# LeadRDRK/ZPack

Hardware: AMD Instinct MI355X
Metric: decompressed GiB/s over all entries; % HBM roofline (higher is better)
Workload: dtype u8; 1 GPU; c2_lz4_64k; entries_per_gpu=100000, entries_total=100000, archive_image_bytes_this_rank=3543588472, archive_image_bytes_all_ranks=3543588472, method=lz4, level=0, class_mix=70/20/5/5 text/records/random/runs, parallelism=one batch per rank, no data-path collective, rehearsal_one_card=False, frames_by=liblz4/libzstd of the image, reference writer call sequence

## Files before the change

### zpack_amd/csrc/xxh3_device.h

```cpp
#pragma once
#include "zpk_device.h"

namespace zpk {

#define ZPK_P32_1 0x9E3779B1U
#define ZPK_P32_2 0x85EBCA77U
#define ZPK_P32_3 0xC2B2AE3DU
#define ZPK_P32_4 0x27D4EB2FU
#define ZPK_P32_5 0x165667B1U
#define ZPK_P64_1 0x9E3779B185EBCA87ULL
#define ZPK_P64_2 0xC2B2AE3D27D4EB4FULL
#define ZPK_P64_3 0x165667B19E3779F9ULL
#define ZPK_P64_4 0x85EBCA77C2B2AE63ULL
#define ZPK_P64_5 0x27D4EB2F165667C5ULL
#define ZPK_PMX_1 0x165667919E3779F9ULL
#define ZPK_PMX_2 0x9FB21C651E98DF25ULL

__device__ __constant__ const u8 XXH3_SECRET[192] = {
    0xb8, 0xfe, 0x6c, 0x39, 0x23, 0xa4, 0x4b, 0xbe, 0x7c, 0x01, 0x81, 0x2c, 0xf7, 0x21, 0xad, 0x1c,
    0xde, 0xd4, 0x6d, 0xe9, 0x83, 0x90, 0x97, 0xdb, 0x72, 0x40, 0xa4, 0xa4, 0xb7, 0xb3, 0x67, 0x1f,
    0xcb, 0x79, 0xe6, 0x4e, 0xcc, 0xc0, 0xe5, 0x78, 0x82, 0x5a, 0xd0, 0x7d, 0xcc, 0xff, 0x72, 0x21,
    0xb8, 0x08, 0x46, 0x74, 0xf7, 0x43, 0x24, 0x8e, 0xe0, 0x35, 0x90, 0xe6, 0x81, 0x3a, 0x26, 0x4c,
    0x3c, 0x28, 0x52, 0xbb, 0x91, 0xc3, 0x00, 0xcb, 0x88, 0xd0, 0x65, 0x8b, 0x1b, 0x53, 0x2e, 0xa3,
    0x71, 0x64, 0x48, 0x97, 0xa2, 0x0d, 0xf9, 0x4e, 0x38, 0x19, 0xef, 0x46, 0xa9, 0xde, 0xac, 0xd8,
    0xa8, 0xfa, 0x76, 0x3f, 0xe3, 0x9c, 0x34, 0x3f, 0xf9, 0xdc, 0xbb, 0xc7, 0xc7, 0x0b, 0x4f, 0x1d,
    0x8a, 0x51, 0xe0, 0x4b, 0xcd, 0xb4, 0x59, 0x31, 0xc8, 0x9f, 0x7e, 0xc9, 0xd9, 0x78, 0x73, 0x64,
    0xea, 0xc5, 0xac, 0x83, 0x34, 0xd3, 0xeb, 0xc3, 0xc5, 0x81, 0xa0, 0xff, 0xfa, 0x13, 0x63, 0xeb,
    0x17, 0x0d, 0xdd, 0x51, 0xb7, 0xf0, 0xda, 0x49, 0xd3, 0x16, 0x55, 0x26, 0x29, 0xd4, 0x68, 0x9e,
    0x2b, 0x16, 0xbe, 0x58, 0x7d, 0x47, 0xa1, 0xfc, 0x8f, 0xf8, 0xb8, 0xd1, 0x7a, 0xd0, 0x31, 0xce,
    0x45, 0xcb, 0x3a, 0x8f, 0x95, 0x16, 0x04, 0x28, 0xaf, 0xd7, 0xfb, 0xca, 0xbb, 0x4b, 0x40, 0x7e,
};

__device__ __forceinline__ u64 sec64(int off) { return ld64(XXH3_SECRET + off); }
__device__ __forceinline__ u32 sec32(int off) { return ld32(XXH3_SECRET + off); }

__device__ __forceinline__ u64 mul128_fold64(u64 a, u64 b) { return (a * b) ^ __umul64hi(a, b); }
__device__ __forceinline__ u64 xxh64_avalanche(u64 h)
{
    h ^= h >> 33; h *= ZPK_P64_2; h ^= h >> 29; h *= ZPK_P64_3; h ^= h >> 32; return h;
}
__device__ __forceinline__ u64 xxh3_avalanche(u64 h) { h ^= h >> 37; h *= ZPK_PMX_1; h ^= h >> 32; return h; }
__device__ __forceinline__ u64 bswap64(u64 x) { return __builtin_bswap64(x); }

__device__ __forceinline__ u64 xxh3_mix16(const u8* in, int soff)
{
    return mul128_fold64(ld64(in) ^ sec64(soff), ld64(in + 8) ^ sec64(soff + 8));
}

__device__ inline u64 xxh3_short(const u8* in, u32 len)
{
    if (len == 0) return xxh64_avalanche(sec64(56) ^ sec64(64));
    if (len <= 3) {
        u32 c1 = ld8(in), c2 = ld8(in + (len >> 1)), c3 = ld8(in + len - 1);
        u32 combined = (c1 << 16) | (c2 << 24) | c3 | (len << 8);
        u64 flip = (u64)(sec32(0) ^ sec32(4));
        return xxh64_avalanche((u64)combined ^ flip);
    }
    if (len <= 8) {
        u32 a = ld32(in), b = ld32(in + len - 4);
        u64 flip = sec64(8) ^ sec64(16);
        u64 in64 = (u64)b + ((u64)a << 32);
        u64 h = in64 ^ flip;
        h ^= rotl64(h, 49) ^ rotl64(h, 24);
        h *= ZPK_PMX_2;
        h ^= (h >> 35) + len;
        h *= ZPK_PMX_2;
        return h ^ (h >> 28);
    }
    if (len <= 16) {
        u64 lo = ld64(in) ^ (sec64(24) ^ sec64(32));
        u64 hi = ld64(in + len - 8) ^ (sec64(40) ^ sec64(48));
        u64 acc = len + bswap64(lo) + hi + mul128_fold64(lo, hi);
        return xxh3_avalanche(acc);
    }
    if (len <= 128) {
        u64 acc = (u64)len * ZPK_P64_1;
        if (len > 32) {
            if (len > 64) {
                if (len > 96) {
                    acc += xxh3_mix16(in + 48, 96);
                    acc += xxh3_mix16(in + len - 64, 112);
                }
                acc += xxh3_mix16(in + 32, 64);
                acc += xxh3_mix16(in + len - 48, 80);
            }
            acc += xxh3_mix16(in + 16, 32);
            acc += xxh3_mix16(in + len - 32, 48);
        }
        acc += xxh3_mix16(in, 0);
        acc += xxh3_mix16(in + len - 16, 16);
        return xxh3_avalanche(acc);
    }
    u64 acc = (u64)len * ZPK_P64_1;
    u32 rounds = len / 16;
    for (u32 i = 0; i < 8; i++) acc += xxh3_mix16(in + 16 * i, 16 * (int)i);
    acc = xxh3_avalanche(acc);
    for (u32 i = 8; i < rounds; i++) acc += xxh3_mix16(in + 16 * i, 16 * (int)(i - 8) + 3);
    acc += xxh3_mix16(in + len - 16, 136 - 17);
    return xxh3_avalanche(acc);
}


struct Xxh3Wave {
    u64 a0, a1;
    u64 k0, k1;
    u64 s0, s1;

    __device__ __forceinline__ void init(int lane)
    {
        const int q = lane & 3, s = lane >> 2;
        const u64 init[8] = { ZPK_P32_3, ZPK_P64_1, ZPK_P64_2, ZPK_P64_3, ZPK_P64_4, ZPK_P32_2, ZPK_P64_5, ZPK_P32_1 };
        a0 = q == 0 ? init[0] : q == 1 ? init[2] : q == 2 ? init[4] : init[6];
        a1 = q == 0 ? init[1] : q == 1 ? init[3] : q == 2 ? init[5] : init[7];
        k0 = sec64(8 * s + 16 * q); k1 = sec64(8 * s + 16 * q + 8);
        s0 = sec64(128 + 16 * q);   s1 = sec64(128 + 16 * q + 8);
    }

    static __device__ __forceinline__ void slot(u64 d0, u64 d1, u64 key0, u64 key1, u64& c0, u64& c1)
    {
        u64 x0 = d0 ^ key0, x1 = d1 ^ key1;
        c0 = (u64)(u32)x0 * (u64)(u32)(x0 >> 32) + d1;
        c1 = (u64)(u32)x1 * (u64)(u32)(x1 >> 32) + d0;
    }

    template <int CTRL>
    static __device__ __forceinline__ u64 add_rotated(u64 c)
    {
        const u32 rl = (u32)__builtin_amdgcn_update_dpp(0, (int)(u32)c, CTRL, 0xf, 0xf, false);
        const u32 rh = (u32)__builtin_amdgcn_update_dpp(0, (int)(u32)(c >> 32), CTRL, 0xf, 0xf, false);
        return c + (((u64)rh << 32) | rl);
    }
    static __device__ __forceinline__ u64 add_rows(u64 c)
    {
        const u32 lo = (u32)c, hi = (u32)(c >> 32);
        auto l16 = __builtin_amdgcn_permlane16_swap(lo, lo, false, false);
        auto h16 = __builtin_amdgcn_permlane16_swap(hi, hi, false, false);
        const u64 s = (((u64)h16[0] << 32) | l16[0]) + (((u64)h16[1] << 32) | l16[1]);
        const u32 slo = (u32)s, shi = (u32)(s >> 32);
        auto l32 = __builtin_amdgcn_permlane32_swap(slo, slo, false, false);
        auto h32 = __builtin_amdgcn_permlane32_swap(shi, shi, false, false);
        return (((u64)h32[0] << 32) | l32[0]) + (((u64)h32[1] << 32) | l32[1]);
    }
    template <bool NO_LDS>
    static __device__ __forceinline__ void reduce16(u64& c0, u64& c1)
    {
        if (!NO_LDS) {
            #pragma unroll
            for (int m = 4; m < 64; m <<= 1) { c0 += shfl_xor64(c0, m); c1 += shfl_xor64(c1, m); }
        } else {
            c0 = add_rotated<0x124>(c0); c1 = add_rotated<0x124>(c1);
            c0 = add_rotated<0x128>(c0); c1 = add_rotated<0x128>(c1);
            c0 = add_rows(c0); c1 = add_rows(c1);
        }
    }

    __device__ __forceinline__ void scramble()
    {
        a0 = ((a0 ^ (a0 >> 47)) ^ s0) * ZPK_P32_1;
        a1 = ((a1 ^ (a1 >> 47)) ^ s1) * ZPK_P32_1;
    }

    __device__ __forceinline__ void block(u128 d)
    {
        u64 c0, c1;
        slot(d.lo, d.hi, k0, k1, c0, c1);
        reduce16<false>(c0, c1);
        a0 += c0; a1 += c1;
        scramble();
    }

    __device__ __forceinline__ u64 finish(const u8* p, u32 nstripes, const u8* end, u64 total_len, int lane)
    {
        const int q = lane & 3, s = lane >> 2;
        u64 c0 = 0, c1 = 0;
        if ((u32)s < nstripes) {
            u128 d = ld128(p + 16 * lane);
            slot(d.lo, d.hi, k0, k1, c0, c1);
        } else if (s == 15) {
            u128 d = ld128(end - 64 + 16 * q);
            slot(d.lo, d.hi, sec64(121 + 16 * q), sec64(121 + 16 * q + 8), c0, c1);
        }
        reduce16<false>(c0, c1);
        a0 += c0; a1 += c1;
        u64 t = mul128_fold64(a0 ^ sec64(11 + 16 * q), a1 ^ sec64(11 + 16 * q + 8));
        t += shfl_xor64(t, 1);
        t += shfl_xor64(t, 2);
        return xxh3_avalanche(total_len * ZPK_P64_1 + t);
    }
};

struct Xxh3Lite {
    u64 a0, a1;
    __device__ __forceinline__ void init(int lane)
    {
        Xxh3Wave w; w.init(lane); a0 = w.a0; a1 = w.a1;
    }
    __device__ __forceinline__ void block(u128 d, int lane, lds_cp8 sec = nullptr)
    {
        const int q = lane & 3, s = lane >> 2;
        u64 k0, k1, s0, s1;
        if (sec) {
            k0 = ((const ZPK_LDS u64*)(sec + 8 * s + 16 * q))[0]; k1 = ((const ZPK_LDS u64*)(sec + 8 * s + 16 * q))[1];
            s0 = ((const ZPK_LDS u64*)(sec + 128 + 16 * q))[0];   s1 = ((const ZPK_LDS u64*)(sec + 128 + 16 * q))[1];
        } else { k0 = sec64(8 * s + 16 * q); k1 = sec64(8 * s + 16 * q + 8); s0 = sec64(128 + 16 * q); s1 = sec64(128 + 16 * q + 8); }
        u64 c0, c1;
        Xxh3Wave::slot(d.lo, d.hi, k0, k1, c0, c1);
        Xxh3Wave::reduce16<true>(c0, c1);
        a0 += c0; a1 += c1;
        a0 = ((a0 ^ (a0 >> 47)) ^ s0) * ZPK_P32_1;
        a1 = ((a1 ^ (a1 >> 47)) ^ s1) * ZPK_P32_1;
    }
    __device__ __forceinline__ u64 finish(const u8* p, u32 nstripes, const u8* end, u64 total_len, int lane)
    {
        Xxh3Wave w; w.init(lane); w.a0 = a0; w.a1 = a1;
        return w.finish(p, nstripes, end, total_len, lane);
    }
};

__device__ __forceinline__ u64 xxh3_64_wave(const u8* p, u64 len, int lane)
{
    if (len <= 240) {
        u64 h = 0;
        lane0_guard();
        if (lane == 0) h = xxh3_short(p, (u32)len);
        return uni64(h);
    }
    Xxh3Wave st;
    st.init(lane);
    const u64 nblocks = (len - 1) >> 10;
    const u8* q = p + 16 * lane;
    if (nblocks > 0) {
        const u64 last = nblocks - 1;
        #define XXH3_LD(i) ld128(q + (((i) < last ? (i) : last) << 10))
        u128 a0 = XXH3_LD(0), a1 = XXH3_LD(1);
        for (u64 b = 0; b < nblocks; b += 4) {
            const u128 c0 = XXH3_LD(b + 2), c1 = XXH3_LD(b + 3);
            st.block(a0);
            if (b + 1 < nblocks) st.block(a1);
            a0 = XXH3_LD(b + 4); a1 = XXH3_LD(b + 5);
            if (b + 2 < nblocks) st.block(c0);
            if (b + 3 < nblocks) st.block(c1);
        }
        #undef XXH3_LD
    }
    const u32 nstripes = (u32)(((len - 1) - (nblocks << 10)) >> 6);
    return st.finish(p + (nblocks << 10), nstripes, p + len, len, lane);
}


__device__ inline u32 xxh32_serial(const u8* p, u64 len, u32 seed)
{
    const u8* end = p + len;
    u32 h;
    if (len >= 16) {
        u32 v1 = seed + ZPK_P32_1 + ZPK_P32_2, v2 = seed + ZPK_P32_2, v3 = seed, v4 = seed - ZPK_P32_1;
        do {
            v1 = rotl32(v1 + ld32(p) * ZPK_P32_2, 13) * ZPK_P32_1;
            v2 = rotl32(v2 + ld32(p + 4) * ZPK_P32_2, 13) * ZPK_P32_1;
            v3 = rotl32(v3 + ld32(p + 8) * ZPK_P32_2, 13) * ZPK_P32_1;
            v4 = rotl32(v4 + ld32(p + 12) * ZPK_P32_2, 13) * ZPK_P32_1;
            p += 16;
        } while (p + 16 <= end);
        h = rotl32(v1, 1) + rotl32(v2, 7) + rotl32(v3, 12) + rotl32(v4, 18);
    } else {
        h = seed + ZPK_P32_5;
    }
    h += (u32)len;
    while (p + 4 <= end) { h = rotl32(h + ld32(p) * ZPK_P32_3, 17) * ZPK_P32_4; p += 4; }
    while (p < end) { h = rotl32(h + (u32)ld8(p) * ZPK_P32_5, 11) * ZPK_P32_1; p++; }
    h ^= h >> 15; h *= ZPK_P32_2; h ^= h >> 13; h *= ZPK_P32_3; h ^= h >> 16;
    return h;
}

__device__ __forceinline__ u64 xxh64_round(u64 acc, u64 in) { return rotl64(acc + in * ZPK_P64_2, 31) * ZPK_P64_1; }

__device__ inline u64 xxh64_serial(const u8* p, u64 len, u64 seed)
{
    const u8* end = p + len;
    u64 h;
    if (len >= 32) {
        u64 v1 = seed + ZPK_P64_1 + ZPK_P64_2, v2 = seed + ZPK_P64_2, v3 = seed, v4 = seed - ZPK_P64_1;
        do {
            v1 = xxh64_round(v1, ld64(p)); v2 = xxh64_round(v2, ld64(p + 8));
            v3 = xxh64_round(v3, ld64(p + 16)); v4 = xxh64_round(v4, ld64(p + 24));
            p += 32;
        } while (p + 32 <= end);
        h = rotl64(v1, 1) + rotl64(v2, 7) + rotl64(v3, 12) + rotl64(v4, 18);
        h = (h ^ xxh64_round(0, v1)) * ZPK_P64_1 + ZPK_P64_4;
        h = (h ^ xxh64_round(0, v2)) * ZPK_P64_1 + ZPK_P64_4;
        h = (h ^ xxh64_round(0, v3)) * ZPK_P64_1 + ZPK_P64_4;
        h = (h ^ xxh64_round(0, v4)) * ZPK_P64_1 + ZPK_P64_4;
    } else {
        h = seed + ZPK_P64_5;
    }
    h += len;
    while (p + 8 <= end) { h ^= xxh64_round(0, ld64(p)); h = rotl64(h, 27) * ZPK_P64_1 + ZPK_P64_4; p += 8; }
    if (p + 4 <= end) { h ^= (u64)ld32(p) * ZPK_P64_1; h = rotl64(h, 23) * ZPK_P64_2 + ZPK_P64_3; p += 4; }
    while (p < end) { h ^= (u64)ld8(p) * ZPK_P64_5; h = rotl64(h, 11) * ZPK_P64_1; p++; }
    return xxh64_avalanche(h);
}

}
```

### zpack_amd/csrc/zpk_codec.hip

```cpp
#include <hip/hip_runtime.h>
#include <stdio.h>
#include <stdlib.h>
#include <string.h>
#include <new>
#include <time.h>
#include <pthread.h>
#include <thread>
#include <atomic>
#include <vector>
#include <algorithm>


#include "zpk_device.h"
#include "xxh3_device.h"
#include "xxh3_span.h"
#include "lz4_wave.h"
#include "lx_ring.h"
#ifndef LX_WAVES_PER_SIMD
#define LX_WAVES_PER_SIMD 6
#endif
#include "zstd_wg.h"
#include "zstd_fse4.h"
#include "zstd_ring.h"
#include "lz4_pj.h"
#include "zstd_pj.h"
#include "host_walk.h"

using namespace zpk;

enum { L_NONE = 0, L_ZSTD = 1, L_LZ4 = 2, L_COUNT = 4, N_LISTS = 3, L_LZ4_RUNS = 100 ,
       L_LZ4_GEN = 101  };
enum { C_ZSTD_TWO_STAGE = 9, C_ZSTD_FUSED = 10, C_EXEC_HEAD = 16, C_LEFT_COUNT = 17,
       C_RETRY_LZ4 = 18, C_RETRY_ZSTD = 19,
       C_RETRY_HEAD = 20,
       C_LZ4_LEFT = 21, C_LZ4_LEFT_HEAD = 22,
       C_LZ4_GEN = 3, C_LZ4_GEN_HEAD = 7,
       C_LZ4_HANDED_HEAD = 23, C_LZ4_HANDED = 24,
       C_LZ4_RETRY_HEAD = 25,
       C_ENC_CLASS = 28,
       C_ORDER_SPAN = 26,
       C_ORDER = 32,
       N_COUNTERS = 32 + 96 };
enum { S_LZ4_HANDED = N_LISTS + 5, S_LZ4_GEN = N_LISTS + 6, S_LZ4_GEN_ORDERED = N_LISTS + 7, N_LISTS_ALLOC = N_LISTS + 8 };
#define N_ORDERED 3
__device__ __forceinline__ int order_list_slot(int y) { return y == 0 ? (int)L_ZSTD : y == 1 ? (int)L_LZ4 : (int)S_LZ4_GEN; }
__device__ __forceinline__ int order_count_word(int y) { return y == 0 ? (int)L_ZSTD : y == 1 ? (int)L_LZ4 : (int)C_LZ4_GEN; }
__device__ __forceinline__ int order_out_slot(int y) { return y == 2 ? (int)S_LZ4_GEN_ORDERED : (int)N_LISTS + 3 + y; }


#define ORD_CLASSES 16
__device__ __forceinline__ int order_class(u64 size)
{
    const int lg = 63 - __clzll((long long)(size | 1));
    const int b = 26 - lg;
    return b < 0 ? 0 : (b > ORD_CLASSES - 1 ? ORD_CLASSES - 1 : b);
}
__device__ __forceinline__ int order_fast(u64 size, u64 comp) { return comp * 16 >= size * 15 ? 1 : 0; }
__device__ __forceinline__ bool lz4_header_is_plain(const u8* __restrict__ p, u64 comp_size)
{
    if (comp_size < 11) return false;
    const u32 magic = (u32)p[0] | ((u32)p[1] << 8) | ((u32)p[2] << 16) | ((u32)p[3] << 24), flg = p[4], bd = p[5];
    return magic == 0x184D2204u && (flg & 0xD7u) == 0x40u && (bd & 0x8Fu) == 0 && ((bd >> 4) & 7u) >= 4u;
}
__global__ __launch_bounds__(256) void k_classify(const u8* __restrict__ src, const zpk_decode_desc* __restrict__ desc, u64 n, u64 src_size, u64 dst_size,
                                                  zpk_decode_result* __restrict__ res, u32* __restrict__ lists, u64 list_stride,
                                                  u32* __restrict__ counters)
{
    u64 i = (u64)blockIdx.x * blockDim.x + threadIdx.x;
    const bool live = i < n;
    zpk_decode_desc d; memset(&d, 0, sizeof(d));
    if (live) d = desc[i];
    zpk_decode_result r; r.status = R_OK; r.detail = 0; r.produced = 0; r.hash = 0;
    int list = -1;
    if (!live) list = -1;
    else if (d.comp_size == 0) r.status = R_OK;
    else if (d.dst_capacity < d.uncomp_size) r.status = R_BUFFER_TOO_SMALL;
    else if (d.src_offset + d.comp_size >= src_size || d.src_offset > src_size || d.comp_size > src_size - d.src_offset)
        r.status = R_FILE_OFFSET_INVALID;
    else if (d.dst_offset > dst_size || d.dst_capacity > dst_size - d.dst_offset) { r.status = R_BUFFER_TOO_SMALL; r.detail = 0xBAD0D57u; }
    else if (d.method == ZPK_METHOD_NONE) {
        if (d.uncomp_size > d.comp_size) r.status = R_FILE_SIZE_INVALID;
        else list = L_NONE;
    }
    else if (d.method == ZPK_METHOD_ZSTD) list = L_ZSTD;
    else if (d.method == ZPK_METHOD_LZ4)
        list = d.comp_size < (d.uncomp_size >> 3) ? L_LZ4_RUNS : lz4_header_is_plain(src + d.src_offset, d.comp_size) ? L_LZ4 : L_LZ4_GEN;
    else r.status = R_COMP_METHOD_INVALID;
    if (list >= 0) { r.status = R_DECOMPRESS_FAILED; r.detail = 0xFFFFFFFFu; }
    if (live) res[i] = r;
    const int lane = lane_id();
    {
        const bool dec = list == L_ZSTD || list == L_LZ4 || list == L_LZ4_GEN;
        u32 hi = dec ? (u32)order_class(d.uncomp_size) + 1u : 0u, inv = dec ? (u32)(ORD_CLASSES - order_class(d.uncomp_size)) : 0u;
        #pragma unroll
        for (int m = 1; m < 64; m <<= 1) { const u32 a = (u32)__shfl_xor((int)hi, m, 64), b2 = (u32)__shfl_xor((int)inv, m, 64); hi = a > hi ? a : hi; inv = b2 > inv ? b2 : inv; }
        if (lane == 0 && hi) { atomicMax(&counters[C_ORDER_SPAN], hi - 1u); atomicMax(&counters[C_ORDER_SPAN + 1], inv - 1u); }
    }
    #pragma unroll
    for (int L = 0; L < N_LISTS; L++) {
        const u64 m = __ballot(list == L);
        if (m == 0) continue;
        const int leader = __ffsll((long long)m) - 1;
        u32 base = 0;
        if (lane == leader) base = atomicAdd(&counters[L], (u32)__popcll(m));
        base = (u32)__shfl((int)base, leader, 64);
        if (list == L) lists[(u64)L * list_stride + base + (u32)__popcll(m & ((1ull << lane) - 1))] = (u32)i;
    }
    {
        const u64 m = __ballot(list == L_LZ4_RUNS);
        if (m != 0) {
            const int leader = __ffsll((long long)m) - 1;
            u32 base = 0;
            if (lane == leader) base = atomicAdd(&counters[C_LZ4_LEFT], (u32)__popcll(m));
            base = (u32)__shfl((int)base, leader, 64);
            if (list == L_LZ4_RUNS) lists[(u64)(N_LISTS + 2) * list_stride + base + (u32)__popcll(m & ((1ull << lane) - 1))] = (u32)i;
        }
    }
    {
        const u64 m = __ballot(list == L_LZ4_GEN);
        if (m != 0) {
            const int leader = __ffsll((long long)m) - 1;
            u32 base = 0;
            if (lane == leader) base = atomicAdd(&counters[C_LZ4_GEN], (u32)__popcll(m));
            base = (u32)__shfl((int)base, leader, 64);
            if (list == L_LZ4_GEN) lists[(u64)S_LZ4_GEN * list_stride + base + (u32)__popcll(m & ((1ull << lane) - 1))] = (u32)i;
        }
    }
}

__device__ __forceinline__ bool order_single_class(const u32* counters) { return counters[C_ORDER_SPAN] + counters[C_ORDER_SPAN + 1] == ORD_CLASSES - 1; }
__device__ __forceinline__ void order_wave_rank(int b, int lane, u32& rank, u32& count)
{
    rank = 0; count = 0;
    u64 todo = __ballot(b >= 0);
    while (todo) {
        const int cls = __shfl(b, __ffsll((long long)todo) - 1, 64);
        const u64 m = __ballot(b == cls);
        if (b == cls) { rank = (u32)__popcll(m & ((1ull << lane) - 1)); count = (u32)__popcll(m); }
        todo &= ~m;
    }
}
__global__ __launch_bounds__(256) void k_order_count(const zpk_decode_desc* __restrict__ desc, const u32* __restrict__ lists, u64 list_stride,
                                                     u32* __restrict__ counters, int fast_last)
{
    __shared__ u32 h[ORD_CLASSES];
    const int L = order_list_slot(blockIdx.y);
    const u32 cnt = counters[order_count_word(blockIdx.y)];
    const bool uniform = order_single_class(counters);
    if ((u64)blockIdx.x * 256 >= cnt || (uniform && !fast_last)) return;
    if (threadIdx.x < ORD_CLASSES) h[threadIdx.x] = 0;
    __syncthreads();
    const u64 k = (u64)blockIdx.x * 256 + threadIdx.x;
    const int lane = lane_id();
    int b = -1;
    if (k < cnt) { const zpk_decode_desc& d = desc[lists[(u64)L * list_stride + k]]; b = uniform ? order_fast(d.uncomp_size, d.comp_size) : order_class(d.uncomp_size); }
    u32 rank, count;
    order_wave_rank(b, lane, rank, count);
    if (b >= 0 && rank == 0) atomicAdd(&h[b], count);
    __syncthreads();
    if (threadIdx.x < ORD_CLASSES && h[threadIdx.x]) atomicAdd(&counters[C_ORDER + blockIdx.y * ORD_CLASSES + threadIdx.x], h[threadIdx.x]);
}
__global__ __launch_bounds__(256) void k_order_fill(const zpk_decode_desc* __restrict__ desc, const u32* __restrict__ lists, u64 list_stride,
                                                    u32* __restrict__ all_lists , u32* __restrict__ counters, int fast_last)
{
    __shared__ u32 wcount[4][ORD_CLASSES], base[ORD_CLASSES];
    const int L = order_list_slot(blockIdx.y);
    const u32 cnt = counters[order_count_word(blockIdx.y)];
    u32* const ordered = all_lists + (u64)order_out_slot(blockIdx.y) * list_stride;
    if ((u64)blockIdx.x * 256 >= cnt) return;
    const u64 k = (u64)blockIdx.x * 256 + threadIdx.x;
    const bool uniform = order_single_class(counters);
    if (uniform && !fast_last) { if (k < cnt) ordered[k] = lists[(u64)L * list_stride + k]; return; }
    if (threadIdx.x < 4 * ORD_CLASSES) (&wcount[0][0])[threadIdx.x] = 0;
    __syncthreads();
    const int lane = lane_id(), w = threadIdx.x >> 6;
    u32 e = 0; int b = -1;
    if (k < cnt) { e = lists[(u64)L * list_stride + k]; b = uniform ? order_fast(desc[e].uncomp_size, desc[e].comp_size) : order_class(desc[e].uncomp_size); }
    u32 rank, count;
    order_wave_rank(b, lane, rank, count);
    if (b >= 0 && rank == 0) wcount[w][b] = count;
    __syncthreads();
    if (threadIdx.x < ORD_CLASSES) {
        const int c = threadIdx.x;
        const u32 total = wcount[0][c] + wcount[1][c] + wcount[2][c] + wcount[3][c];
        const u32* const hist = counters + C_ORDER + blockIdx.y * ORD_CLASSES;
        u32 before = 0;
        for (int j = 0; j < c; j++) before += hist[j];
        base[c] = total ? before + atomicAdd(&counters[C_ORDER + N_ORDERED * ORD_CLASSES + blockIdx.y * ORD_CLASSES + c], total) : 0;
    }
    __syncthreads();
    if (b >= 0) {
        u32 at = base[b] + rank;
        for (int j = 0; j < w; j++) at += wcount[j][b];
        ordered[at] = e;
    }
}

__device__ __forceinline__ bool my_slot(const u32* counters, int list, u32& idx)
{
    idx = uni((u32)(((u64)blockIdx.x * blockDim.x + threadIdx.x) >> 6));
    return idx < uni(counters[list]);
}

__device__ __forceinline__ void finish_entry(const zpk_decode_desc& d, zpk_decode_result* res, u32 e, int status, u32 detail,
                                             u64 produced, const u8* out, int lane)
{
    u64 h = 0;
    lane0_guard();
    if (status == R_OK) {
        wave_mem_fence();
#ifndef ZPK_ABL_NOHASH
        h = xxh3_64_wave(out, d.uncomp_size, lane);
#endif
        if (h != d.expect_hash && !(d.flags & ZPK_DF_SKIP_HASH)) status = R_FILE_HASH_MISMATCH;
    }
    lane0_guard();
    if (lane == 0) {
        zpk_decode_result r; r.status = status; r.detail = detail; r.produced = produced; r.hash = h;
        res[e] = r;
    }
}

__global__ __launch_bounds__(256) void k_stored(const u8* __restrict__ src, const zpk_decode_desc* __restrict__ desc,
                                                u8* __restrict__ dst, zpk_decode_result* __restrict__ res,
                                                const u32* __restrict__ list, const u32* __restrict__ counters)
{
    const int lane = lane_id();
    u32 idx;
    if (my_slot(counters, L_NONE, idx)) {
        const u32 e = uni(list[idx]);
        const zpk_decode_desc d = desc[e];
        const u8* in = uni_ptr(src + d.src_offset);
        u8* out = uni_ptr(dst + d.dst_offset);
        const u64 len = uni64(d.uncomp_size);
        u64 h;
        if (len <= 240) {
            for (u64 i = lane; i < len; i += WAVE) st8(out + i, ld8(in + i));
            h = 0;
            lane0_guard();
            if (lane == 0) h = xxh3_short(in, (u32)len);
            h = uni64(h);
        } else {
            Xxh3Wave st; st.init(lane);
            const u64 nblocks = (len - 1) >> 10;
            const u8* q = in + 16 * lane;
            u8* o = out + 16 * lane;
            u128 cur = {0, 0};
            if (nblocks) cur = ld128(q);
            for (u64 b = 0; b < nblocks; b++) {
                u128 nxt = {0, 0};
                if (b + 1 < nblocks) nxt = ld128(q + ((b + 1) << 10));
                st128(o + (b << 10), cur);
                st.block(cur);
                cur = nxt;
            }
            const u64 done = nblocks << 10;
            for (u64 i = done + lane; i < len; i += WAVE) st8(out + i, ld8(in + i));
            const u32 nstripes = (u32)(((len - 1) - done) >> 6);
            h = st.finish(in + done, nstripes, in + len, len, lane);
        }
        int status = R_OK;
        if (!(d.flags & ZPK_DF_SKIP_HASH) && h != d.expect_hash) status = R_FILE_HASH_MISMATCH;
        lane0_guard();
        if (lane == 0) {
            zpk_decode_result r; r.status = status; r.detail = 0; r.produced = len; r.hash = h;
            res[e] = r;
        }
    }
}

__device__ __forceinline__ void lz4_stats_out(u64* __restrict__ dbg, u32 e, const SeqStats& stt, u64 t_all, int lane)
{
#ifdef ZPK_STATS
    if (dbg && lane == 0) {
        u64* g = dbg + (u64)e * 8;
        g[0] = stt.t_parse; g[1] = stt.t_lit; g[2] = stt.t_dep; g[3] = stt.t_rounds;
        g[4] = ((u64)stt.batches << 32) | stt.rounds; g[5] = ((u64)stt.coops << 32) | stt.asm_batches; g[6] = SEQ_T() - t_all;
        g[7] = ((u64)stt.fix_iters << 32) | stt.chunks;
#ifdef ZPK_STATS_PARSE
        g[0] = stt.t_stage; g[1] = stt.t_walk1; g[2] = stt.t_fix; g[3] = stt.t_emit; g[4] = stt.t_tok;
        g[5] = ((u64)stt.hops_first << 32) | stt.hops_fix; g[6] = stt.slow_hops;
#endif
    }
#else
    (void)dbg; (void)e; (void)stt; (void)t_all; (void)lane;
#endif
}

template <int COOP>
__device__ __forceinline__ void lz4_entry_wave(Lz4WaveShared& shw, const u8* __restrict__ src, const u8* read_lo, const u8* read_hi,
                                               const zpk_decode_desc* __restrict__ desc, u8* dst, zpk_decode_result* __restrict__ res,
                                               u32 e, u32* __restrict__ counters, u64* __restrict__ dbg, u32* __restrict__ retry_list,
                                               u32 wd_scale, int lane)
{
    const zpk_decode_desc d = desc[e];
    const u8* in = uni_ptr(src + d.src_offset);
    u8* out = uni_ptr(dst + d.dst_offset);
    Watchdog wd; wd.arm(uni64(d.comp_size) + uni64(d.dst_capacity), wd_scale);
    SeqStats stt = {};
    const u64 t_all = SEQ_T(); (void)t_all;
    DecodeOut o = lz4f_decode_wave<COOP>(shw, wd, stt, in, uni64(d.comp_size), read_lo, read_hi, out, uni64(d.dst_capacity), lane);
    lz4_stats_out(dbg, e, stt, t_all, lane);
    if (wd.fired && retry_list) {
        lane0_guard();
        if (lane == 0) retry_list[atomicAdd(&counters[C_RETRY_LZ4], 1u)] = e;
        return;
    }
    int status = R_OK;
    if (o.rc == D_MALFORMED) status = R_DECOMPRESS_FAILED;
    else if (o.rc == D_TRUNCATED) status = o.produced < d.dst_capacity ? R_FILE_INCOMPLETE : R_BUFFER_TOO_SMALL;
    else if (o.rc == D_DST_FULL) status = R_BUFFER_TOO_SMALL;
    finish_entry(d, res, e, status, wd.fired ? 0xDEADu : (u32)(-o.rc), o.produced, out, lane);
}

__device__ __forceinline__ void lz4_entry_plain(Lz4WaveShared& shw, const u8* __restrict__ src, const u8* read_hi,
                                                const zpk_decode_desc* __restrict__ desc, u8* dst, zpk_decode_result* __restrict__ res,
                                                u32 e, u32* __restrict__ counters, u64* __restrict__ dbg, u32* __restrict__ retry_list,
                                                u32* __restrict__ handed_list, u32 wd_scale, int lane)
{
    const zpk_decode_desc& d = desc[e];
    const u8* in = uni_ptr(src + d.src_offset);
    u8* out = uni_ptr(dst + d.dst_offset);
    Watchdog wd; wd.arm(uni64(d.comp_size) + uni64(d.dst_capacity), wd_scale);
    SeqStats stt = {};
    const u64 t_all = SEQ_T(); (void)t_all;
    const bool done = lz4f_plain_wave<0>(shw, wd, stt, in, uni64(d.comp_size), read_hi, out, uni64(d.dst_capacity), uni64(d.uncomp_size), lane);
    lz4_stats_out(dbg, e, stt, t_all, lane);
    if (!done) {
        lane0_guard();
        if (lane == 0) {
            if (wd.fired) retry_list[atomicAdd(&counters[C_RETRY_LZ4], 1u)] = e;
            else handed_list[atomicAdd(&counters[C_LZ4_HANDED], 1u)] = e;
        }
        return;
    }
    finish_entry(d, res, e, R_OK, 0u, uni64(d.uncomp_size), out, lane);
}

__global__ __launch_bounds__(64, 8) void k_lz4_wave(const u8* __restrict__ src, const u8* read_hi,
                                                  const zpk_decode_desc* __restrict__ desc, u8* dst,
                                                  zpk_decode_result* __restrict__ res, const u32* __restrict__ list,
                                                  u32* __restrict__ counters, u32* __restrict__ retry_list, u32* __restrict__ handed_list
#ifdef ZPK_DEVELOPER
                                                  , u64* __restrict__ dbg, u32 wd_scale
#endif
                                                  )
{
#ifndef ZPK_DEVELOPER
    const u32 wd_scale = 1u;
    u64* const dbg = nullptr;
#endif
    const int lane = lane_id();
    __shared__ Lz4WaveShared shw;
    u32 idx;
    if (my_slot(counters, L_LZ4, idx))
        lz4_entry_plain(shw, src, read_hi, desc, dst, res, uni(list[idx]), counters, dbg, retry_list, handed_list, wd_scale, lane);
}

#ifdef ZPK_DEVELOPER
__global__ __launch_bounds__(256) void k_lz4_hand_all(const u32* __restrict__ list, u32* __restrict__ counters, u32* __restrict__ handed_list)
{
    const u64 i = (u64)blockIdx.x * blockDim.x + threadIdx.x;
    if (i < counters[L_LZ4]) handed_list[atomicAdd(&counters[C_LZ4_HANDED], 1u)] = list[i];
}
#endif

#define LZ4_GENERAL_GRID_MAX 8192u
__global__ __launch_bounds__(64, 8) void k_lz4_general(const u8* __restrict__ src, const u8* read_lo, const u8* read_hi,
                                                     const zpk_decode_desc* __restrict__ desc, u8* dst,
                                                     zpk_decode_result* __restrict__ res, const u32* __restrict__ list,
                                                     u32* __restrict__ counters, u64* __restrict__ dbg, u32* __restrict__ retry_list, u32 wd_scale)
{
    const int lane = lane_id();
    __shared__ Lz4WaveShared shw;
    const u32 n_slots = uni(counters[C_LZ4_GEN]);
    if (n_slots == 0) return;
    for (;;) {
        lane0_guard();
        u32 v = 0;
        if (lane == 0) v = atomicAdd(&counters[C_LZ4_GEN_HEAD], 1u);
        const u32 idx = uni(v);
        lane0_guard();
        if (idx >= n_slots) break;
        lz4_entry_wave<0>(shw, src, read_lo, read_hi, desc, dst, res, uni(list[idx]), counters, dbg, retry_list, wd_scale, lane);
    }
}

__global__ __launch_bounds__(64, 8) void k_lz4_retry(const u8* __restrict__ src, const u8* read_lo, const u8* read_hi,
                                                   const zpk_decode_desc* __restrict__ desc, u8* dst,
                                                   zpk_decode_result* __restrict__ res, const u32* __restrict__ lists, u64 list_stride,
                                                   u32* __restrict__ counters, u64* __restrict__ dbg, int gen_slot)
{
    const int lane = lane_id();
    __shared__ Lz4WaveShared shw;
    for (int k = 0; k < 3; k++) {
        const int count_word = k == 0 ? (int)C_LZ4_GEN : k == 1 ? (int)C_LZ4_HANDED : (int)C_RETRY_LZ4;
        const int head_word = k == 0 ? (int)C_LZ4_GEN_HEAD : k == 1 ? (int)C_LZ4_HANDED_HEAD : (int)C_LZ4_RETRY_HEAD;
        const u32* const list = lists + (u64)(k == 0 ? gen_slot : k == 1 ? (int)S_LZ4_HANDED : (int)N_LISTS) * list_stride;
        const u32 n_slots = uni(counters[count_word]);
        if (n_slots == 0 || uni(counters[head_word]) >= n_slots) continue;
        for (;;) {
            lane0_guard();
            u32 v = 0;
            if (lane == 0) v = atomicAdd(&counters[head_word], 1u);
            const u32 idx = uni(v);
            lane0_guard();
            if (idx >= n_slots) break;
            lz4_entry_wave<2>(shw, src, read_lo, read_hi, desc, dst, res, uni(list[idx]), counters, dbg, nullptr, (u32)ZPK_WATCHDOG_RETRY_SCALE, lane);
        }
    }
}

#define LZ4_LEFT_GRID_MAX 8192u
#ifndef LZ4_LEFT_WAVES
#define LZ4_LEFT_WAVES 8
#endif
__global__ __launch_bounds__(64, LZ4_LEFT_WAVES) void k_lz4_left(const u8* __restrict__ src, const u8* read_lo, const u8* read_hi,
                                                  const zpk_decode_desc* __restrict__ desc, u8* dst,
                                                  zpk_decode_result* __restrict__ res, const u32* __restrict__ list,
                                                  u32* __restrict__ counters, u64* __restrict__ dbg, u32* __restrict__ retry_list, u32 wd_scale)
{
    const int lane = lane_id();
    __shared__ Lz4WaveShared shw;
    const u32 n_slots = uni(counters[C_LZ4_LEFT]);
    if (n_slots == 0) return;
    for (;;) {
        lane0_guard();
        u32 v = 0;
        if (lane == 0) v = atomicAdd(&counters[C_LZ4_LEFT_HEAD], 1u);
        const u32 idx = uni(v);
        lane0_guard();
        if (idx >= n_slots) break;
        lz4_entry_wave<2>(shw, src, read_lo, read_hi, desc, dst, res, uni(list[idx]), counters, dbg, retry_list, wd_scale, lane);
    }
}

#define ZSTD_EXEC_GRID_MAX 4096
#ifndef ZSTD_EXEC_WAVES
#define ZSTD_EXEC_WAVES 4
#endif
#ifndef ZSTD_EXEC_DIRECT
#define ZSTD_EXEC_RING 1
#endif
__global__ __launch_bounds__(ZSTD_WG_THREADS, ZSTD_EXEC_WAVES) void k_zstd_exec(const u8* __restrict__ src, const zpk_decode_desc* __restrict__ desc,
                                                               u8* dst, zpk_decode_result* __restrict__ res,
                                                               const u32* __restrict__ list, u32* __restrict__ counters,
                                                               u8* __restrict__ lit_scratch, const u64* __restrict__ arena,
                                                               u32* __restrict__ zstate, u32* __restrict__ leftover, u64* __restrict__ dbg)
{
    const int lane = lane_id();
    const u32 nz = uni(counters[L_ZSTD]);
    if (nz == 0) return;
#ifndef ZSTD_EXEC_RING
    __shared__ __attribute__((aligned(16))) u8 sh_raw[ZSTD_SHARED_EXEC_BYTES];
    ZstdShared& sh = *(ZstdShared*)sh_raw;
    if (threadIdx.x == 0) { sh.defaults_built = 0; sh.huf_valid = 0; }
#else
    __shared__ ZstdRingShared sh;
    if (threadIdx.x == 0) sh.huf_valid = 0;
#endif
    __syncthreads();
    u8* lit = lit_scratch + (u64)blockIdx.x * ZSTD_LIT_SCRATCH;
    for (;;) {
        lane0_guard();
        u32 v = 0;
        if (lane == 0) v = atomicAdd(&counters[C_EXEC_HEAD], 1u);
        const u32 idx = uni(v);
        lane0_guard();
        if (idx >= nz) break;
        const u32 e = uni(list[idx]);
        if (uni(zstate[e]) != 1u) {
            lane0_guard();
            if (lane == 0) leftover[atomicAdd(&counters[C_LEFT_COUNT], 1u)] = e;
            lane0_guard();
            continue;
        }
        const zpk_decode_desc d = desc[e];
        const u8* in = uni_ptr(src + d.src_offset);
        u8* out = uni_ptr(dst + d.dst_offset);
        const u64* const pre = arena + (((u64)d.dst_offset + 7) >> 3);
        Watchdog wd; wd.arm(uni64(d.comp_size) + uni64(d.dst_capacity));
#ifndef ZSTD_EXEC_RING
#ifdef ZPK_STATS
        ZstdStats zs = {};
        const u64 t_all = SEQ_T();
        DecodeOut o = zstd_decode_wave<true>(sh, wd, in, uni64(d.comp_size), out, uni64(d.dst_capacity), lit, lane, &zs, pre);
        const u64 t_dec = SEQ_T();
#else
        (void)dbg;
        DecodeOut o = zstd_decode_wave<true>(sh, wd, in, uni64(d.comp_size), out, uni64(d.dst_capacity), lit, lane, nullptr, pre);
#endif
        bool ok = o.rc == D_OK;
        u64 h = 0;
        lane0_guard();
        if (ok) {
            wave_mem_fence();
    #ifndef ZPK_ABL_NOHASH
        h = xxh3_64_wave(out, d.uncomp_size, lane);
#endif
            ok = h == d.expect_hash || (d.flags & ZPK_DF_SKIP_HASH);
        }
        const int ok_status = R_OK;
#ifdef ZPK_STATS
        if (dbg && lane == 0) {
            u64* g = dbg + (u64)e * 16;
            g[0] = zs.t_lit; g[1] = zs.t_tab; g[2] = zs.t_fse; g[3] = zs.t_exec; g[4] = zs.nseq; g[5] = zs.nblk; g[6] = t_dec - t_all; g[7] = SEQ_T() - t_dec;
        }
#endif
#else
        (void)dbg;
        struct { int rc; u64 produced; } o;
        const LxResult xr = zstd_ring_decode_wave(sh, wd, in, uni64(d.comp_size), out, uni64(d.dst_capacity), uni64(d.uncomp_size), lit, pre, lane,
                                                   dbg ? dbg + (u64)e * 16 : nullptr);
        o.rc = xr.rc == LX_OK ? D_OK : -(0x100 + xr.rc); o.produced = xr.produced;
        const u64 h = xr.hash;
        const bool ok = xr.rc == LX_OK && xr.produced == uni64(d.uncomp_size);
        const int ok_status = (h == d.expect_hash || (d.flags & ZPK_DF_SKIP_HASH)) ? R_OK : R_FILE_HASH_MISMATCH;
#endif
        lane0_guard();
        if (lane == 0) {
            if (ok) {
                zpk_decode_result r; r.status = ok_status; r.detail = 0; r.produced = o.produced; r.hash = h;
                res[e] = r;
                zstate[e] = 2u;
                atomicAdd(&counters[C_ZSTD_TWO_STAGE], 1u);
            } else {
                leftover[atomicAdd(&counters[C_LEFT_COUNT], 1u)] = e;
                atomicAdd(&counters[14], 1u); counters[15] = ((u32)(-o.rc) & 0xFFFFu);
            }
        }
    }
}

__global__ __launch_bounds__(ZSTD_WG_THREADS, 3) void k_zstd(const u8* __restrict__ src, const zpk_decode_desc* __restrict__ desc,
                                                          u8* dst, zpk_decode_result* __restrict__ res,
                                                          const u32* __restrict__ list, u32* __restrict__ counters,
                                                          u8* __restrict__ lit_scratch, u64* __restrict__ dbg, int count_word,
                                                          int head_word, u32* __restrict__ retry_list, int retry_word, u32 wd_scale)
{
    const int lane = lane_id();
    const u32 nz = uni(counters[count_word]);
    if (nz == 0) return;
    __shared__ ZstdShared sh;
    if (threadIdx.x == 0) { sh.defaults_built = 0; sh.huf_valid = 0; }
    __syncthreads();
    u8* lit = lit_scratch + (u64)blockIdx.x * ZSTD_LIT_SCRATCH;
    for (;;) {
        lane0_guard();
        u32 v = 0;
        if (lane == 0) v = atomicAdd(&counters[head_word], 1u);
        const u32 idx = uni(v);
        lane0_guard();
        if (idx >= nz) break;
        const u32 e = uni(list[idx]);
        const zpk_decode_desc d = desc[e];
        const u8* in = uni_ptr(src + d.src_offset);
        u8* out = uni_ptr(dst + d.dst_offset);
        Watchdog wd; wd.arm(uni64(d.comp_size) + uni64(d.dst_capacity), wd_scale);
#ifdef ZPK_STATS
        ZstdStats zs = {};
        const u64 t_all = SEQ_T();
        DecodeOut o = zstd_decode_wave<false>(sh, wd, in, uni64(d.comp_size), out, uni64(d.dst_capacity), lit, lane, &zs);
        if (dbg && lane == 0) {
            u64* g = dbg + (u64)e * 8;
            g[0] = zs.t_lit; g[1] = zs.t_tab; g[2] = zs.t_fse; g[3] = zs.t_exec; g[4] = zs.nseq; g[5] = zs.nblk; g[6] = SEQ_T() - t_all; g[7] = 0;
        }
#else
        (void)dbg;
        DecodeOut o = zstd_decode_wave<false>(sh, wd, in, uni64(d.comp_size), out, uni64(d.dst_capacity), lit, lane);
#endif
        int status = o.rc == D_OK ? R_OK : R_DECOMPRESS_FAILED;
        if (wd.fired && retry_list) {
            lane0_guard();
            if (lane == 0) retry_list[atomicAdd(&counters[retry_word], 1u)] = e;
            lane0_guard();
            continue;
        }
        finish_entry(d, res, e, status, wd.fired ? 0xDEADu : (u32)(-o.rc), o.produced, out, lane);
        lane0_guard();
        if (lane == 0) atomicAdd(&counters[C_ZSTD_FUSED], 1u);
    }
}

__global__ __launch_bounds__(256) void k_hash(const u8* __restrict__ src, const u64* __restrict__ offsets,
                                              const u64* __restrict__ sizes, u64 n, u64* __restrict__ hashes)
{
    const int lane = lane_id();
    const u64 w = uni64(((u64)blockIdx.x * blockDim.x + threadIdx.x) >> 6);
    if (w < n) {
        u64 h = xxh3_64_wave(uni_ptr(src + offsets[w]), uni64(sizes[w]), lane);
        lane0_guard();
        if (lane == 0) hashes[w] = h;
    }
}


#define ZPK_DEC_SPLIT_MIN_DEFAULT (256ull << 10)
#define ZPK_ENC_SPLIT_MIN_DEFAULT (2ull << 20)
#define ZPK_ENC_PIECE (512u << 10)
#ifndef ZPK_PJ_CHUNK_BLOCKS
#define ZPK_PJ_CHUNK_BLOCKS 512u
#endif
#define ZPK_PJ_MAX_CHUNKS 64u
struct zpk_codec {
    int device = 0;
    hipStream_t stream = nullptr;
    pthread_mutex_t mu;
    u32* d_counters = nullptr;
    u32* d_lists = nullptr;      u64 list_cap = 0;
    u8*  d_lit = nullptr;        u64 lit_cap = 0;
    u8*  d_src = nullptr;        u64 src_cap = 0;
    u8*  h_pin[2] = {nullptr, nullptr};
    hipEvent_t pin_ev[2] = {nullptr, nullptr};
    hipStream_t s_up = nullptr, s_dn = nullptr;
    hipStream_t s_side = nullptr;
    hipEvent_t ev_fork = nullptr, ev_join = nullptr;
    void* d_pj_blocks = nullptr; u64 pj_blocks_cap = 0;
    void* d_pj_recs = nullptr;   u64 pj_recs_cap = 0;
    void* d_pj_masks = nullptr;  u64 pj_masks_cap = 0;
    void* d_pj_S = nullptr;      u64 pj_S_cap = 0;
    u32*  d_pj_flags = nullptr;
    u8*   h_bigsrc = nullptr; u64 h_bigsrc_cap = 0;
    u8*   d_big1 = nullptr;
    u32   zpj_last_err = 0;
    void* d_zpj_blocks = nullptr; u64 zpj_blocks_cap = 0;
    void* d_zpj_aux = nullptr;    u64 zpj_aux_cap = 0;
    void* d_zpj_pos = nullptr;    u64 zpj_pos_cap = 0;
    hipStream_t s_left = nullptr;
    hipEvent_t ev_lfork = nullptr, ev_ljoin = nullptr;
    volatile u32* h_seen = nullptr;
    hipEvent_t pipe_ev[2 * 64] = {};
    u8*  d_dst = nullptr;        u64 dst_cap = 0;
    void* d_desc = nullptr;      u64 desc_cap = 0;
    void* d_res = nullptr;       u64 res_cap = 0;
    u64* d_dbg = nullptr;        u64 dbg_cap = 0;
    u64* d_seq = nullptr;        u64 seq_cap = 0;
    u8*  d_pack = nullptr;       u64 pack_cap = 0;
    u8*  d_packed = nullptr;     u64 packed_cap = 0;
    u8*  d_packoff = nullptr;    u64 packoff_cap = 0;
// ... 1301 lines not shown
```

Measured before the change: 646.2 GiB/s.

## Restructure wave XXH3 to hash four blocks per iteration with row-wise reduction

The wave-level XXH3 hash now maps each 16-lane row to a different 1 KiB block, so one group iteration covers four blocks. Each lane accumulates products locally, reduces within its row using lean DPP adds, and broadcasts the four row sums with ds_bpermute before folding them into the accumulator in order. This replaces the per-block full-wave xor-shuffle reduction. In the LZ4 paths the secret keys are staged once into the LDS stage buffer instead of being reloaded. The aim is to cut reduction and synchronisation cost on the hash that runs after each decoded entry. The cost is extra LDS traffic, more complex tail handling for partial groups, and reuse of the shared stage buffer, which must not be live at that point.

```diff
diff --git a/zpack_amd/csrc/xxh3_device.h b/zpack_amd/csrc/xxh3_device.h
--- a/zpack_amd/csrc/xxh3_device.h
+++ b/zpack_amd/csrc/xxh3_device.h
@@ -106,15 +106,20 @@
     u64 k0, k1;
     u64 s0, s1;
 
-    __device__ __forceinline__ void init(int lane)
-    {
-        const int q = lane & 3, s = lane >> 2;
+    __device__ __forceinline__ void init_acc(int lane)
+    {
+        const int q = lane & 3;
         const u64 init[8] = { ZPK_P32_3, ZPK_P64_1, ZPK_P64_2, ZPK_P64_3, ZPK_P64_4, ZPK_P32_2, ZPK_P64_5, ZPK_P32_1 };
         a0 = q == 0 ? init[0] : q == 1 ? init[2] : q == 2 ? init[4] : init[6];
         a1 = q == 0 ? init[1] : q == 1 ? init[3] : q == 2 ? init[5] : init[7];
+        s0 = sec64(128 + 16 * q);   s1 = sec64(128 + 16 * q + 8);
+    }
+    __device__ __forceinline__ void init_keys(int lane)
+    {
+        const int q = lane & 3, s = lane >> 2;
         k0 = sec64(8 * s + 16 * q); k1 = sec64(8 * s + 16 * q + 8);
-        s0 = sec64(128 + 16 * q);   s1 = sec64(128 + 16 * q + 8);
-    }
+    }
+    __device__ __forceinline__ void init(int lane) { init_acc(lane); init_keys(lane); }
 
     static __device__ __forceinline__ void slot(u64 d0, u64 d1, u64 key0, u64 key1, u64& c0, u64& c1)
     {
@@ -123,12 +128,18 @@
         c1 = (u64)(u32)x1 * (u64)(u32)(x1 >> 32) + d0;
     }
 
-    template <int CTRL>
+    static __device__ __forceinline__ u64 pair64(u32 lo, u32 hi)
+    {
+        u64 v = ((u64)hi << 32) | lo;
+        asm volatile("" : "+v"(v));
+        return v;
+    }
+    template <int CTRL, bool LEAN = false>
     static __device__ __forceinline__ u64 add_rotated(u64 c)
     {
-        const u32 rl = (u32)__builtin_amdgcn_update_dpp(0, (int)(u32)c, CTRL, 0xf, 0xf, false);
-        const u32 rh = (u32)__builtin_amdgcn_update_dpp(0, (int)(u32)(c >> 32), CTRL, 0xf, 0xf, false);
-        return c + (((u64)rh << 32) | rl);
+        const u32 rl = (u32)__builtin_amdgcn_update_dpp(0, (int)(u32)c, CTRL, 0xf, 0xf, LEAN);
+        const u32 rh = (u32)__builtin_amdgcn_update_dpp(0, (int)(u32)(c >> 32), CTRL, 0xf, 0xf, LEAN);
+        return c + (LEAN ? pair64(rl, rh) : (((u64)rh << 32) | rl));
     }
     static __device__ __forceinline__ u64 add_rows(u64 c)
     {
@@ -167,6 +178,50 @@
         reduce16<false>(c0, c1);
         a0 += c0; a1 += c1;
         scramble();
+    }
+
+    static __device__ __forceinline__ void quad_keys(int lane, int it, u64& key0, u64& key1)
+    {
+        const int off = 32 * it + 8 * ((lane >> 2) & 3) + 16 * (lane & 3);
+        key0 = sec64(off); key1 = sec64(off + 8);
+    }
+    static __device__ __forceinline__ void quad_keys(lds_cp8 sec, int lane, int it, u64& key0, u64& key1)
+    {
+        const ZPK_LDS u64* w = (const ZPK_LDS u64*)(sec + 8 * ((lane >> 2) & 3) + 16 * (lane & 3)) + 4 * it;
+        key0 = w[0]; key1 = w[1];
+    }
+    static __device__ __forceinline__ void stage_secret(lds_p8 sec, int lane)
+    {
+        wave_mem_fence();
+        if (lane < 12) lds_st128(sec + 16 * lane, ld128(XXH3_SECRET + 16 * lane));
+        wave_mem_fence();
+    }
+    static __device__ __forceinline__ void quad_slot(u128 d, u64 key0, u64 key1, u64& t0, u64& t1)
+    {
+        u64 c0, c1;
+        slot(d.lo, d.hi, key0, key1, c0, c1);
+        t0 += c0; t1 += c1;
+    }
+    static __device__ __forceinline__ void row_sum(u64& t0, u64& t1)
+    {
+        t0 = add_rotated<0x124, true>(t0); t1 = add_rotated<0x124, true>(t1);
+        t0 = add_rotated<0x128, true>(t0); t1 = add_rotated<0x128, true>(t1);
+    }
+    template <int R>
+    static __device__ __forceinline__ u64 row_bcast_lds(u64 v, int l15x4)
+    {
+        const u32 lo = (u32)__builtin_amdgcn_ds_bpermute(l15x4 + 64 * R, (int)(u32)v);
+        const u32 hi = (u32)__builtin_amdgcn_ds_bpermute(l15x4 + 64 * R, (int)(u32)(v >> 32));
+        return pair64(lo, hi);
+    }
+    __device__ __forceinline__ void fold(u64 S0, u64 S1) { a0 += S0; a1 += S1; scramble(); }
+    __device__ __forceinline__ void fold_rows(u64 t0, u64 t1, u32 n, int lane)
+    {
+        const int l15x4 = 4 * (lane & 15);
+        fold(row_bcast_lds<0>(t0, l15x4), row_bcast_lds<0>(t1, l15x4));
+        if (n > 1) fold(row_bcast_lds<1>(t0, l15x4), row_bcast_lds<1>(t1, l15x4));
+        if (n > 2) fold(row_bcast_lds<2>(t0, l15x4), row_bcast_lds<2>(t1, l15x4));
+        if (n > 3) fold(row_bcast_lds<3>(t0, l15x4), row_bcast_lds<3>(t1, l15x4));
     }
 
     __device__ __forceinline__ u64 finish(const u8* p, u32 nstripes, const u8* end, u64 total_len, int lane)
@@ -217,7 +272,8 @@
     }
 };
 
-__device__ __forceinline__ u64 xxh3_64_wave(const u8* p, u64 len, int lane)
+template <bool LDS_KEYS = false>
+__device__ __forceinline__ u64 xxh3_64_wave(const u8* p, u64 len, int lane, lds_p8 sec = nullptr)
 {
     if (len <= 240) {
         u64 h = 0;
@@ -226,23 +282,42 @@
         return uni64(h);
     }
     Xxh3Wave st;
-    st.init(lane);
-    const u64 nblocks = (len - 1) >> 10;
-    const u8* q = p + 16 * lane;
+    st.init_acc(lane);
+    const u64 nblocks = uni64((len - 1) >> 10);
     if (nblocks > 0) {
-        const u64 last = nblocks - 1;
-        #define XXH3_LD(i) ld128(q + (((i) < last ? (i) : last) << 10))
-        u128 a0 = XXH3_LD(0), a1 = XXH3_LD(1);
-        for (u64 b = 0; b < nblocks; b += 4) {
-            const u128 c0 = XXH3_LD(b + 2), c1 = XXH3_LD(b + 3);
-            st.block(a0);
-            if (b + 1 < nblocks) st.block(a1);
-            a0 = XXH3_LD(b + 4); a1 = XXH3_LD(b + 5);
-            if (b + 2 < nblocks) st.block(c0);
-            if (b + 3 < nblocks) st.block(c1);
+        const u64 lastg = (nblocks - 1) >> 2;
+        const u32 nlast = (((u32)nblocks - 1u) & 3u) + 1u;
+        const u32 row = (u32)lane >> 4, l16 = 16u * ((u32)lane & 15u);
+        u64 kc[4][2] = {};
+        if (LDS_KEYS) Xxh3Wave::stage_secret(sec, lane);
+        else { Xxh3Wave::quad_keys(lane, 0, kc[0][0], kc[0][1]); Xxh3Wave::quad_keys(lane, 1, kc[1][0], kc[1][1]);
+               Xxh3Wave::quad_keys(lane, 2, kc[2][0], kc[2][1]); Xxh3Wave::quad_keys(lane, 3, kc[3][0], kc[3][1]); }
+        #define XXH3_SLOT(d, it) do { u64 k0_ = kc[it][0], k1_ = kc[it][1]; if (LDS_KEYS) Xxh3Wave::quad_keys((lds_cp8)sec, lane, it, k0_, k1_); \
+                                      Xxh3Wave::quad_slot(d, k0_, k1_, t0, t1); } while (0)
+        const u32 off_full = (row << 10) + l16, off_last = ((row < nlast ? row : nlast - 1u) << 10) + l16;
+        #define XXH3_LD(g, it) ld128(p + ((g) << 12) + ((g) == lastg ? off_last : off_full) + 256u * (it))
+        u128 a0 = XXH3_LD((u64)0, 0), a1 = XXH3_LD((u64)0, 1);
+        #pragma clang loop unroll(disable)
+        for (u64 g = 0; g <= lastg; g++) {
+            const u128 c0 = XXH3_LD(g, 2), c1 = XXH3_LD(g, 3);
+            __builtin_amdgcn_sched_barrier(0);
+            u64 t0 = 0, t1 = 0;
+            XXH3_SLOT(a0, 0);
+            XXH3_SLOT(a1, 1);
+            const u64 gn = g < lastg ? g + 1 : lastg;
+            asm volatile("" : "+v"(t0), "+v"(t1));
+            __builtin_amdgcn_sched_barrier(0);
+            a0 = XXH3_LD(gn, 0); a1 = XXH3_LD(gn, 1);
+            __builtin_amdgcn_sched_barrier(0);
+            XXH3_SLOT(c0, 2);
+            XXH3_SLOT(c1, 3);
+            Xxh3Wave::row_sum(t0, t1);
+            st.fold_rows(t0, t1, g == lastg ? nlast : 4u, lane);
         }
         #undef XXH3_LD
-    }
+        #undef XXH3_SLOT
+    }
+    st.init_keys(lane);
     const u32 nstripes = (u32)(((len - 1) - (nblocks << 10)) >> 6);
     return st.finish(p + (nblocks << 10), nstripes, p + len, len, lane);
 }
diff --git a/zpack_amd/csrc/zpk_codec.hip b/zpack_amd/csrc/zpk_codec.hip
--- a/zpack_amd/csrc/zpk_codec.hip
+++ b/zpack_amd/csrc/zpk_codec.hip
@@ -202,15 +202,16 @@
     return idx < uni(counters[list]);
 }
 
+template <bool LDS_KEYS = false>
 __device__ __forceinline__ void finish_entry(const zpk_decode_desc& d, zpk_decode_result* res, u32 e, int status, u32 detail,
-                                             u64 produced, const u8* out, int lane)
+                                             u64 produced, const u8* out, int lane, lds_p8 sec = nullptr)
 {
     u64 h = 0;
     lane0_guard();
     if (status == R_OK) {
         wave_mem_fence();
 #ifndef ZPK_ABL_NOHASH
-        h = xxh3_64_wave(out, d.uncomp_size, lane);
+        h = xxh3_64_wave<LDS_KEYS>(out, d.uncomp_size, lane, sec);
 #endif
         if (h != d.expect_hash && !(d.flags & ZPK_DF_SKIP_HASH)) status = R_FILE_HASH_MISMATCH;
     }
@@ -310,7 +311,7 @@
     if (o.rc == D_MALFORMED) status = R_DECOMPRESS_FAILED;
     else if (o.rc == D_TRUNCATED) status = o.produced < d.dst_capacity ? R_FILE_INCOMPLETE : R_BUFFER_TOO_SMALL;
     else if (o.rc == D_DST_FULL) status = R_BUFFER_TOO_SMALL;
-    finish_entry(d, res, e, status, wd.fired ? 0xDEADu : (u32)(-o.rc), o.produced, out, lane);
+    finish_entry<true>(d, res, e, status, wd.fired ? 0xDEADu : (u32)(-o.rc), o.produced, out, lane, to_lds_rw(shw.stage));
 }
 
 __device__ __forceinline__ void lz4_entry_plain(Lz4WaveShared& shw, const u8* __restrict__ src, const u8* read_hi,
@@ -334,7 +335,7 @@
         }
         return;
     }
-    finish_entry(d, res, e, R_OK, 0u, uni64(d.uncomp_size), out, lane);
+    finish_entry<true>(d, res, e, R_OK, 0u, uni64(d.uncomp_size), out, lane, to_lds_rw(shw.stage));
 }
 
 __global__ __launch_bounds__(64, 8) void k_lz4_wave(const u8* __restrict__ src, const u8* read_hi,
```

New measurement: 661.1 GiB/s (median of 6 runs). 2.3% higher.
